# sk4161/EgoScaler

Measured on AMD Instinct MI355X. Metric: clips/sec/GPU (8-frame 224^2, 16-token text) fwd+bwd, higher is better.
Workload: dtype bf16

## Files before the change

egoscaler_amd/csrc/gemm_fast.hip:

```cpp
#include "common.h"
#include <mutex>
#include <queue>
#include <unordered_map>
#include <vector>

#define FT_BK 64

struct FastArgs {
    const bf16_t* A; const bf16_t* B; void* C; const bf16_t* bias; const void* residual;
    int M, N, K;
    long long lda, ldb, ldc, ldr;
    float alpha; int accumulate; int act;
    int tiles_m, tiles_n;
    int splitk; float* ws;
    int full_tm, full_tiles, tail_s;
    int epi; void* C2; long long ldc2;
    int* tickets;
};

typedef __attribute__((address_space(3))) void lds_void;
typedef __attribute__((address_space(1))) const void gbl_void;

__device__ __forceinline__ void glds16(const bf16_t* g, bf16_t* lds_wave_base) {
    __builtin_amdgcn_global_load_lds((gbl_void*)g, (lds_void*)lds_wave_base, 16, 0, 0);
}

template <typename TC, int MT, bool RES, bool ACC>
__device__ __forceinline__ void gemm_epilogue_interior(const FastArgs& g, const f32x4 (&acc)[4][MT], const int mb, const int nb, const int lane) {
    TC* cp = reinterpret_cast<TC*>(g.C) + (long long)(mb + (lane & 15)) * g.ldc + nb + (lane >> 4) * 4;
    const TC* rp = RES ? reinterpret_cast<const TC*>(g.residual) + (long long)(mb + (lane & 15)) * g.ldr + nb + (lane >> 4) * 4 : nullptr;
    const long long cstep = 16 * g.ldc, rstep = 16 * g.ldr;
#pragma unroll
    for (int i = 0; i < MT; ++i) {
#pragma unroll
        for (int j = 0; j < 4; ++j) {
            f32x4 v = acc[j][i];
            if (sizeof(TC) == 2) {
                if (RES) {
                    const u32x2 rr = *reinterpret_cast<const u32x2*>(rp + j * 16);
                    v[0] += __uint_as_float(rr[0] << 16); v[1] += __uint_as_float(rr[0] & 0xFFFF0000u);
// ... 86 lines not shown
                    o[0] = (uint32_t)f2bf(v[0]) | ((uint32_t)f2bf(v[1]) << 16);
                    o[1] = (uint32_t)f2bf(v[2]) | ((uint32_t)f2bf(v[3]) << 16);
                    *reinterpret_cast<u32x2*>(cp) = o;
                } else {
                    f32x4 o = {v[0], v[1], v[2], v[3]};
                    if (rp) o += *reinterpret_cast<const f32x4*>(rp);
                    if (g.accumulate) o += *reinterpret_cast<const f32x4*>(cp);
                    *reinterpret_cast<f32x4*>(cp) = o;
                }
            } else {
#pragma unroll
                for (int r = 0; r < 4; ++r) {
                    if (n + r >= g.N) continue;
                    float x = v[r];
                    if (rp) x += Cvt<TC>::ld(rp + r);
                    if (g.accumulate) x += Cvt<TC>::ld(cp + r);
                    Cvt<TC>::st(cp + r, x);
                }
            }
        }
    }
}

template <typename TC, int BM, int BN, int NS>
__global__ __launch_bounds__((BM / 64) * (BN / 64) * 64, NS == 2 ? 2 : ((BM * BN == 256 * 128) ? 4 : 3))
void gemm_nt_bf16_kernel(FastArgs g) {
    constexpr int MT = 4;
    constexpr int WN = BN / 64, NW = (BM / 64) * WN;
    constexpr int A_PW = BM / 8 / NW, B_PW = BN / 8 / NW;
    constexpr int STAGE = (BM + BN) * FT_BK;
    constexpr bool PF = NS == 2;
    __shared__ __attribute__((aligned(16))) bf16_t smem[NS * STAGE];
    bf16_t* sA = smem;
    bf16_t* sB = smem + BM * FT_BK;
    const int lane = threadIdx.x & 63;
    const int wave = __builtin_amdgcn_readfirstlane(threadIdx.x >> 6);

    const int nwg = g.tiles_m * g.tiles_n;
    int bid = blockIdx.x;
    {
        const int xcd = bid & 7, q = nwg >> 3, r = nwg & 7;
        bid = (xcd < r ? xcd * (q + 1) : r * (q + 1) + (xcd - r) * q) + (bid >> 3);
    }
    const int per_group = 8 * g.tiles_n;
    const int grp = bid / per_group, first_tm = grp * 8;
    const int gsz = (g.tiles_m - first_tm) < 8 ? (g.tiles_m - first_tm) : 8;
// ... 451 lines not shown
                            swiglu_bwd_elem(bf2f(f2bf(v[r])), gv, uv, og[r], ou[r]);
                        }
                        u32x2 o;
                        o[0] = (uint32_t)f2bf(og[0]) | ((uint32_t)f2bf(og[1]) << 16);
                        o[1] = (uint32_t)f2bf(og[2]) | ((uint32_t)f2bf(og[3]) << 16);
                        *reinterpret_cast<u32x2*>(pg) = o;
                        o[0] = (uint32_t)f2bf(ou[0]) | ((uint32_t)f2bf(ou[1]) << 16);
                        o[1] = (uint32_t)f2bf(ou[2]) | ((uint32_t)f2bf(ou[3]) << 16);
                        *reinterpret_cast<u32x2*>(pg + 64) = o;
                    }
#pragma unroll
                for (int it = 0; it < 8; ++it) {
                    const int m = mb + sp * 32 + it * 4 + lr;
                    const u32x4 v = *reinterpret_cast<const u32x4*>(ws3 + (it * 4 + lr) * 272 + ch * 16);
                    if (m < g.M) *reinterpret_cast<u32x4*>(C + (long long)m * g.ldc + 2 * nb + ch * 8) = v;
                }
            }
#undef P8_GU_FETCH
            GSTAMP(4)
            GSTAMP(5)
            GSTAMP_FLUSH
            return;
        }
#pragma unroll
        for (int pass = 0; pass < 2; ++pass) {
#pragma unroll
            for (int ii = 0; ii < 4; ++ii)
#pragma unroll
                for (int j = 0; j < 4; ++j) {
                    const f32x4 v = acc[j][4 * pass + ii];
                    u32x2 o;
                    o[0] = (uint32_t)f2bf(v[0]) | ((uint32_t)f2bf(v[1]) << 16);
                    o[1] = (uint32_t)f2bf(v[2]) | ((uint32_t)f2bf(v[3]) << 16);
                    *reinterpret_cast<u32x2*>(wb + (ii * 16 + (lane & 15)) * 144 + (j * 16 + (lane >> 4) * 4) * 2) = o;
                }
#pragma unroll
            for (int it = 0; it < 8; ++it) {
                const int r = it * 8 + (lane >> 3), ch = lane & 7;
                const u32x4 v = *reinterpret_cast<const u32x4*>(wb + r * 144 + ch * 16);
                const int m = mb + pass * 64 + r;
                if (m < g.M) *reinterpret_cast<u32x4*>(C + (long long)m * g.ldc + nb + ch * 8) = v;
            }
            if (g.epi == 1) {
                bf16_t* C2 = reinterpret_cast<bf16_t*>(g.C2);
#pragma unroll
                for (int ii = 0; ii < 4; ++ii)
#pragma unroll
                    for (int j = 0; j < 2; ++j) {
                        const f32x4 vg = acc[j][4 * pass + ii], vu = acc[j + 2][4 * pass + ii];
                        float o4[4];
#pragma unroll
                        for (int r = 0; r < 4; ++r) {
                            const float gg = bf2f(f2bf(vg[r])), uu = bf2f(f2bf(vu[r]));
                            const float a = bf2f(f2bf(gg * (1.0f / (1.0f + __expf(-gg)))));
                            o4[r] = a * uu;
                        }
                        u32x2 o;
                        o[0] = (uint32_t)f2bf(o4[0]) | ((uint32_t)f2bf(o4[1]) << 16);
// ... 282 lines not shown
                            swiglu_bwd_elem(bf2f(f2bf(v[r])), gv, uv, og[r], ou[r]);
                        }
                        u32x2 o;
                        o[0] = (uint32_t)f2bf(og[0]) | ((uint32_t)f2bf(og[1]) << 16);
                        o[1] = (uint32_t)f2bf(og[2]) | ((uint32_t)f2bf(og[3]) << 16);
                        *reinterpret_cast<u32x2*>(pg) = o;
                        o[0] = (uint32_t)f2bf(ou[0]) | ((uint32_t)f2bf(ou[1]) << 16);
                        o[1] = (uint32_t)f2bf(ou[2]) | ((uint32_t)f2bf(ou[3]) << 16);
                        *reinterpret_cast<u32x2*>(pg + 64) = o;
                    }
                }
#pragma unroll
                for (int it = 0; it < 8; ++it) {
                    if (sp * 32 + it * 4 >= 16 * TL_NB) continue;
                    const int m = mb + sp * 32 + it * 4 + lr;
                    const u32x4 v = *reinterpret_cast<const u32x4*>(ws3 + (it * 4 + lr) * 272 + ch * 16);
                    if (m < g.M) *reinterpret_cast<u32x4*>(C + (long long)m * g.ldc + 2 * nb + ch * 8) = v;
                }
            }
#undef TL_GU_FETCH
            return;
        }
        char* wb = smem + wave * (64 * 144);
#pragma unroll
        for (int pass = 0; pass < 3; ++pass) {
            const int nblk = (TL_NB - 4 * pass) < 4 ? (TL_NB - 4 * pass) : 4;
#pragma unroll
            for (int ii = 0; ii < 4; ++ii) {
                if (ii >= nblk) continue;
#pragma unroll
                for (int j = 0; j < 4; ++j) {
                    const f32x4 v = acc[j][4 * pass + ii];
                    u32x2 o;
                    o[0] = (uint32_t)f2bf(v[0]) | ((uint32_t)f2bf(v[1]) << 16);
                    o[1] = (uint32_t)f2bf(v[2]) | ((uint32_t)f2bf(v[3]) << 16);
                    *reinterpret_cast<u32x2*>(wb + (ii * 16 + (lane & 15)) * 144 + (j * 16 + (lane >> 4) * 4) * 2) = o;
                }
            }
#pragma unroll
            for (int it = 0; it < 8; ++it) {
                const int r = it * 8 + (lane >> 3), ch = lane & 7;
                if (it * 8 >= nblk * 16) continue;
                const u32x4 v = *reinterpret_cast<const u32x4*>(wb + r * 144 + ch * 16);
                const int m = mb + pass * 64 + r;
                const int ncol = TBK ? n0 + 128 * (ch >> 2) + 32 * wc + (ch & 3) * 8 : nb + ch * 8;
                if (m < g.M) *reinterpret_cast<u32x4*>(C + (long long)m * g.ldc + ncol) = v;
            }
            if (g.epi == 1) {
                bf16_t* C2 = reinterpret_cast<bf16_t*>(g.C2);
#pragma unroll
                for (int ii = 0; ii < 4; ++ii) {
                    if (ii >= nblk) continue;
#pragma unroll
                    for (int j = 0; j < 2; ++j) {
                        const f32x4 vg = acc[j][4 * pass + ii], vu = acc[j + 2][4 * pass + ii];
                        float o4[4];
#pragma unroll
                        for (int r = 0; r < 4; ++r) {
                            const float gg = bf2f(f2bf(vg[r])), uu = bf2f(f2bf(vu[r]));
                            const float a = bf2f(f2bf(gg * (1.0f / (1.0f + __expf(-gg)))));
                            o4[r] = a * uu;
// ... 566 lines not shown
    if (sc.P > 0 && sc.Gr > sc.P) sc.Gr = sc.P;
    if (sc.Gr >= 8) sc.Gr &= ~7;
    sc.tickets = (int*)d->workspace;
    sc.slabs = (float*)((char*)d->workspace + 4096);
    return true;
}
static int launch_p8(const egomi_gemm_desc* d, FastArgs& g, const P8Sched& sc, hipStream_t s) {
    g.tiles_m = (d->M + 255) / 256; g.tiles_n = (d->N + 255) / 256;
    g.splitk = 1; g.ws = nullptr; g.full_tm = g.tiles_m; g.full_tiles = g.tiles_m * g.tiles_n; g.tail_s = 1;
    const long long T = (long long)g.tiles_m * g.tiles_n;
    const int grid = T < sc.G ? (sc.Gr > 0 ? sc.Gr : 1) : sc.G;
    if (d->c_dtype == EGOMI_BF16) EGOMI_LAUNCH(gemm_nt_bf16_p8_kernel<bf16_t>, dim3(grid), dim3(512), 0, s, g, sc);
    else if (d->c_dtype == EGOMI_F32) EGOMI_LAUNCH(gemm_nt_bf16_p8_kernel<float>, dim3(grid), dim3(512), 0, s, g, sc);
    else return EGOMI_E_UNSUPPORTED;
    return egomi_launch_status();
}

static int g_tall_mode = -1;
extern "C" int egomi_gemm_set_tall(int mode) { g_tall_mode = mode < 0 ? -1 : (mode > 2 ? 2 : mode); return EGOMI_OK; }
static bool tall_form(const egomi_gemm_desc* d) {
    if (g_tall_mode < 0) { const char* e = getenv("EGOMI_GEMM_TALL"); g_tall_mode = e ? atoi(e) : 1; if (g_tall_mode < 0 || g_tall_mode > 2) g_tall_mode = 1; }
    const int mode = g_tall_mode;
    if (!mode) return false;
    if (d->epilogue != EGOMI_EPI_NONE && d->epilogue != EGOMI_EPI_SLABS && d->epilogue != EGOMI_EPI_SWIGLU && d->epilogue != EGOMI_EPI_SWIGLU_BWD) return false;
    if ((d->M & 7) || (d->N & 7) || d->M < TL_BM || d->N < 256 || d->K < 2048 || d->split_k > 1) return false;
    if ((long long)d->M * d->lda >= (1ll << 31) || (long long)d->N * d->ldb >= (1ll << 31)) return false;
    if (d->c_dtype != EGOMI_BF16 && d->c_dtype != EGOMI_F32) return false;
    if (mode == 2) return true;
    const int ncu = p8_cus();
    const long long tn = (d->N + 255) / 256;
    const long long t256 = (long long)((d->M + 255) / 256) * tn, t352 = (long long)((d->M + TL_BM - 1) / TL_BM) * tn;
    const int rem = (int)(t256 % ncu);
    const double c256 = (double)(t256 / ncu) + (rem ? (rem * 2 <= ncu && d->workspace ? 0.28 + 0.85 * rem / ncu : 1.0) : 0.0);
    const double c352 = 1.31 * (double)((t352 + ncu - 1) / ncu);
    return c352 < 0.98 * c256;
}
static int launch_tall(const egomi_gemm_desc* d, FastArgs& g, hipStream_t s, hipEvent_t t0, hipEvent_t t1) {
    g.tiles_m = (d->M + TL_BM - 1) / TL_BM; g.tiles_n = (d->N + 255) / 256;
    g.splitk = 1; g.ws = nullptr; g.tickets = nullptr;
    if (g.epi == EGOMI_EPI_SLABS) g.epi = 0;
    static int gdepth = -1;
    if (gdepth < 0) { const char* e = getenv("EGOMI_TALL_GROUP"); gdepth = e ? atoi(e) : 8; if (gdepth < 1) gdepth = 8; }
    g.full_tm = gdepth;
    const int nwg = g.tiles_m * g.tiles_n;
    if (t0) (void)hipEventRecord(t0, s);
    if (d->c_dtype == EGOMI_BF16) EGOMI_LAUNCH((gemm_nt_bf16_tall_kernel<bf16_t, false>), dim3(nwg), dim3(512), 0, s, g);
    else EGOMI_LAUNCH((gemm_nt_bf16_tall_kernel<float, false>), dim3(nwg), dim3(512), 0, s, g);
// ... 147 lines not shown
    const int esz = d->c_dtype == EGOMI_BF16 ? 2 : 4;
    egomi_gemm_desc d1 = *d;
    d1.N = Na;
    FastArgs g1 = g;
    g1.N = Na;
    int rc = launch_tall(&d1, g1, s, t0, nullptr);
    if (rc != EGOMI_OK) return rc;
    egomi_gemm_desc d2 = *d;
    FastArgs g2 = g;
    d2.N = g2.N = d->N - Na;
    d2.B = g2.B = (const bf16_t*)d->B + (long long)Na * d->ldb;
    const long long ccol = d->epilogue == EGOMI_EPI_SWIGLU_BWD ? 2ll * Na : (long long)Na;
    d2.C = g2.C = (char*)d->C + ccol * esz;
    if (d->residual) d2.residual = g2.residual = (const char*)d->residual + (long long)Na * esz;
    if (d->epilogue == EGOMI_EPI_SWIGLU) d2.C2 = g2.C2 = (char*)d->C2 + (long long)(Na / 2) * 2;
    if (d->epilogue == EGOMI_EPI_SWIGLU_BWD) d2.C2 = g2.C2 = (char*)d->C2 + 2ll * Na * 2;
    return launch_8phase(&d2, g2, s, nullptr, nullptr, t1);
}

static bool slabs_form_ok(const egomi_gemm_desc* d) {
    return !d->bias && !d->residual && !d->accumulate && d->act == 0 && d->alpha == 1.0f && d->workspace && d->M <= 512 && (d->N & 3) == 0;
}

extern thread_local hipEvent_t egomi_time_start_, egomi_time_stop_;

int egomi_gemm_fast_try(const egomi_gemm_desc* d0, hipStream_t s) {
    const hipEvent_t t0 = egomi_time_start_, t1 = egomi_time_stop_;
    egomi_time_start_ = egomi_time_stop_ = nullptr;
    if (!fast_applicable(d0)) return 1;
    egomi_gemm_desc dl = *d0;
    const egomi_gemm_desc* d = &dl;
    FastArgs g;
    g.A = (const bf16_t*)d->A; g.B = (const bf16_t*)d->B; g.C = d->C; g.bias = (const bf16_t*)d->bias; g.residual = d->residual;
    g.M = d->M; g.N = d->N; g.K = d->K; g.lda = d->lda; g.ldb = d->ldb; g.ldc = d->ldc; g.ldr = d->ldr;
    g.alpha = d->alpha; g.accumulate = d->accumulate; g.act = d->act; g.tickets = nullptr;
    g.epi = d->epilogue; g.C2 = d->C2; g.ldc2 = d->ldc2;
    const int tc = tile_choice(d);
    if (tc == 8 && (d->epilogue == EGOMI_EPI_NONE || d->epilogue == EGOMI_EPI_SLABS) && tall_form(d)) {
        if (d->epilogue == EGOMI_EPI_SLABS && (d->bias || d->accumulate || d->act != 0 || d->alpha != 1.0f || d->c_dtype != EGOMI_BF16)) return EGOMI_E_UNSUPPORTED;
        return launch_tall(d, g, s, t0, t1);
    }
    if (d->epilogue == EGOMI_EPI_SLABS && tc == 8) {
        if (d->bias || d->accumulate || d->act != 0 || d->alpha != 1.0f || d->c_dtype != EGOMI_BF16 || (d->N & 7) ||
            (long long)d->M * d->lda >= (1ll << 31) || (long long)d->N * d->ldb >= (1ll << 31)) return EGOMI_E_UNSUPPORTED;
        if (dl.ws_tickets_zeroed && dl.workspace) {
            if (dl.workspace_bytes > 4096) { dl.workspace = (char*)dl.workspace + 4096; dl.workspace_bytes -= 4096; }
            else { dl.workspace = nullptr; dl.workspace_bytes = 0; }
        }
        g.epi = 0;
        return launch_8phase(d, g, s, nullptr, t0, t1, true);
    }
    if (d->epilogue == EGOMI_EPI_SLABS) {
        if (!slabs_form_ok(d) || tc != 1) return EGOMI_E_UNSUPPORTED;
        if (dl.ws_tickets_zeroed && dl.workspace) {
            if (dl.workspace_bytes > 4096) { dl.workspace = (char*)dl.workspace + 4096; dl.workspace_bytes -= 4096; }
            else return EGOMI_E_UNSUPPORTED;
        }
        g.epi = 0;
        return launch_fast<128, 128>(d, g, s);
    }
// ... 34 lines not shown
```

egoscaler_amd/decode.py:

```python
import ctypes
import os

import torch

from . import lora, ops
from ._lib import c_p, c_i, c_f, c_i64, call
from .ops import P, S, dt


def kv_append(k, v, ld, kc, vc, B, Sq, H, hd, Smax, pos0):
    call("egomi_kv_append", P(k), P(v), c_i64(ld), P(kc), P(vc), c_i(B), c_i(Sq), c_i(H), c_i(hd), c_i(Smax), c_i(pos0), c_i(dt(k.dtype)), S())


def attn_decode(q, ld_q, kc, vc, key_mask, out, B, H, hd, Smax, T_len, scale):
    call("egomi_attn_decode", P(q), c_i64(ld_q), P(kc), P(vc), P(key_mask), c_i64(key_mask.stride(0) if key_mask is not None else 0),
         P(out), c_i64(out.stride(0)), c_i(B), c_i(H), c_i(hd), c_i(Smax), c_i(T_len), c_f(scale), c_i(dt(q.dtype)), S())


def kv_append_fp8(k, v, ld, kc, vc, ks, vs, B, Sq, H, hd, Smax, pos0):
    call("egomi_kv_append_fp8", P(k), P(v), c_i64(ld), P(kc), P(vc), P(ks), P(vs), c_i(B), c_i(Sq), c_i(H), c_i(hd), c_i(Smax), c_i(pos0),
         c_i(dt(k.dtype)), S())


def attn_decode_fp8(q, ld_q, kc, vc, ks, vs, key_mask, out, B, H, hd, Smax, T_len, scale):
    call("egomi_attn_decode_fp8", P(q), c_i64(ld_q), P(kc), P(vc), P(ks), P(vs), P(key_mask), c_i64(key_mask.stride(0) if key_mask is not None else 0),
         P(out), c_i64(out.stride(0)), c_i(B), c_i(H), c_i(hd), c_i(Smax), c_i(T_len), c_f(scale), c_i(dt(q.dtype)), S())


def kv8_quantize(x):
    x = x.float()
# ... 283 lines not shown
        if seed is None:
            seed = int(torch.randint(0, 2 ** 62, (1,)).item())
        self.rng.copy_(torch.tensor([int(seed), 0], dtype=torch.int64))
        self.done_buf.zero_()
        self.done = self.done_buf if eos is not None else None
        kw = dict(repetition_penalty=float(repetition_penalty or 1.0), temperature=float(temperature or 1.0), top_k=int(top_k or 0),
                  top_p=float(1.0 if top_p is None else top_p), do_sample=bool(do_sample), rng=self.rng, eos=eos, pad=pad)

        def steps():
            for t in range(T_new):
                sample_rows(self.lg, sc_buf[t], self.seq, S0 + t, 0, self.tok.view(-1), self.done, draw=t, **kw)
                if t + 1 < T_new:
                    self.step(S0 + t)
        if not use_graph:
            steps()
        else:
            key = (S0, T_new, kw["repetition_penalty"], kw["temperature"], kw["top_k"], kw["top_p"], kw["do_sample"], eos, pad)
            g = self._graphs.get(key)
            if g is None:
                g = torch.cuda.CUDAGraph()
                side = torch.cuda.Stream()
                side.wait_stream(torch.cuda.current_stream())
                with torch.cuda.stream(side):
                    with torch.cuda.graph(g, stream=side):
                        steps()
                torch.cuda.current_stream().wait_stream(side)
                self._graphs[key] = g
            g.replay()
            self.graph = g
        self.pos = S0 + T_new
        return self.seq, sc_buf

    def greedy(self, T_new, use_graph=True, keep_scores=True):
        S0 = self.pos
        scores = [] if keep_scores else None
        if not use_graph:
            for t in range(T_new):
                if keep_scores:
                    scores.append(self.lg.float().clone())
                argmax_rows(self.lg, self.tok.view(-1), self.seq, S0 + t)
                if t + 1 < T_new:
                    self.step(S0 + t)
            self.pos = S0 + T_new
            return self.seq, scores
        sc_buf = torch.zeros(T_new, self.B, self.lg.shape[1], dtype=torch.float32, device=self.eng.device) if keep_scores else None
        g = torch.cuda.CUDAGraph()
        side = torch.cuda.Stream()
        side.wait_stream(torch.cuda.current_stream())
        with torch.cuda.stream(side):
            with torch.cuda.graph(g, stream=side):
                for t in range(T_new):
                    if keep_scores:
                        ops.cast(self.lg, torch.float32, out=sc_buf[t])
                    argmax_rows(self.lg, self.tok.view(-1), self.seq, S0 + t)
                    if t + 1 < T_new:
                        self.step(S0 + t)
        torch.cuda.current_stream().wait_stream(side)
        g.replay()
        self.graph = g
        self.pos = S0 + T_new
        return self.seq, ([sc_buf[t] for t in range(T_new)] if keep_scores else None)

    def _beam_buffers(self):
        R, Smax, dev = self.B, self.Smax, self.eng.device
        z = lambda *s, dtype: torch.zeros(*s, dtype=dtype, device=dev)
        self.kv_row = z(R, Smax, dtype=torch.int32)
        self.fin_seq = z(R, Smax, dtype=torch.int64)
        self.bidx = z(R, Smax, dtype=torch.int32)
        self.fin_bidx = z(R, Smax, dtype=torch.int32)
        self.run_score, self.fin_score = z(R, dtype=torch.float32), z(R, dtype=torch.float32)
        self.fin_flag, self.heur = z(R, dtype=torch.int32), z(R // self.nb, dtype=torch.int32)
        self.ctl = z(8, dtype=torch.int32)
        self._cands = {}
# ... 34 lines not shown
        kw = dict(repetition_penalty=float(repetition_penalty or 1.0), temperature=float(temperature or 1.0), top_k=int(top_k or 0),
                  top_p=float(1.0 if top_p is None else top_p), min_keep=max(2, n_eos + 1), do_sample=bool(do_sample))
        es = early_stopping if early_stopping == "never" else bool(early_stopping)

        def steps():
            for t in range(T_new):
                beam_rows(self.lg, nb if t == 0 else 1, R, nb, sc_buf[t], self.seq_buf, S0 + t, rng=self.rng, draw=t, run_score=self.run_score,
                          cand_key=cands[0], cand_score=cands[1], cand_tok=cands[2], ctl=self.ctl, **kw)
                beam_update(Bi, nb, V, cands[0], cands[1], cands[2], S0, S0 + t, max_len, eos, float(length_penalty), es, self.seq_buf,
                            self.fin_seq, self.bidx, self.fin_bidx, self.kv_row, self.run_score, self.fin_score, self.fin_flag, self.heur,
                            self.tok.view(-1), self.ctl)
                if t + 1 < T_new:
                    self.step(S0 + t)
        if not use_graph:
            steps()
        else:
            key = ("beam", S0, T_new, nb, float(length_penalty), es, eos, pad, tuple(sorted(kw.items())))
            g = self._graphs.get(key)
            if g is None:
                g = torch.cuda.CUDAGraph()
                side = torch.cuda.Stream()
                side.wait_stream(torch.cuda.current_stream())
                with torch.cuda.stream(side):
                    with torch.cuda.graph(g, stream=side):
                        steps()
                torch.cuda.current_stream().wait_stream(side)
                self._graphs[key] = g
            g.replay()
            self.graph = g
        self.pos = S0 + T_new
        n_iter = int(self.ctl[1])
        nrs = int(num_return_sequences)
        rows = (torch.arange(Bi, device=dev)[:, None] * nb + torch.arange(nrs, device=dev)[None, :]).reshape(-1)
        bidx = self.fin_bidx[rows, :T_new]
        lgen = int((bidx >= 0).sum(1).max()) if T_new > 0 else 0
        return (self.fin_seq[rows, :S0 + lgen].clone(), self.fin_score[rows].clone(), sc_buf[:n_iter].clone(), bidx[:, :lgen].long())
```

egoscaler_amd/engine.py:

```python
import os
from typing import Dict

import torch

from . import lora, ops
from .config import EgoDims


class Workspace:

    def __init__(self, device):
        self.device = device
        self.bufs: Dict[str, torch.Tensor] = {}

    def get(self, name, shape, dtype, zero=False):
        t = self.bufs.get(name)
        shape = tuple(int(s) for s in shape)
        if t is None or t.shape != shape or t.dtype != dtype:
            t = torch.empty(shape, dtype=dtype, device=self.device)
            self.bufs[name] = t
            if zero:
                t.zero_()
        elif zero:
            t.zero_()
# ... 7 lines not shown
    def __init__(self, dims: EgoDims, params: Dict[str, torch.Tensor], device, dtype):
        self.dims, self.w, self.device, self.dtype = dims, params, device, dtype
        self.ws = Workspace(device)
        self.w8 = None
        self.prepared = False
        self.prepare_epoch = 0
        self.lm_wT, self.lm_wT_stale, self.lm_wT_ver = None, True, None
        self.param_ref = {}
        self.grad_fresh = set()
        self._xt_last = {}
        self.main_grad: Dict[str, torch.Tensor] = {}
        self.layer_flat: Dict[int, torch.Tensor] = {}
        self.trainable: Dict[str, bool] = {}
        self.ctx = None
        self.grad_sync = None
        self.pb_drop_override = None
        self.reduced_grad = {}
        self.layer_offs = {}
        self._direct, self._direct_done = None, set()
        self.layer_final_hook = None
        self.param_events = {}
        self.use_fused_attention = True
        self.use_fused_swiglu = os.environ.get("EGOMI_NO_FUSED_SWIGLU", "0") != "1"
        self.use_tail_fuse = os.environ.get("EGOMI_NO_TAIL_FUSE", "0") != "1"
        self.use_tn = os.environ.get("EGOMI_GEMM_TN", "1") != "0"
        self.pb_trainer = None
        self.defer_splice_check = False
        self.pending_splice = None
        self.pb_train_mode = False
        self.prepared_bn_stale = False
        self.fold_stale = False
        self.lora = None
        self.lora_version = 0
        self._lora_ws = None

    @staticmethod
    def param_group_of(name):
        if name.startswith("model.layers."):
            return int(name.split(".")[2])
        if name == "model.embed_tokens.weight":
            return "embed"
        if name in ("model.norm.weight", "lm_head.weight"):
            return "post"
        return "pre"

    def wait_params(self, key):
# ... 323 lines not shown
            Wl, bl = w[f"model.point_proj.{2 * nh}.weight"], w[f"model.point_proj.{2 * nh}.bias"]
            feats_proj = ops.mm(cur, Wl, bias=bl, out=ws.get("pp_out", (Bc * Pn, d), T))
            sp, err, cloud_idx = ops.splice_scan(input_ids, tok, Pn, Bc)
            pending_err = self._stash_splice_err(err)
            start_pos = sp
            if save:
                ctx["pp_acts"] = acts
        if save:
            ctx["start_pos"], ctx["cloud_idx"], ctx["n_clouds"] = start_pos, cloud_idx, Bc
            ctx["has_points"] = feats_proj is not None
        x = ws.get("x_emb", (B, S, d), T) if not save else torch.empty(B, S, d, dtype=T, device=self.device)
        self.wait_params("embed")
        ops.embed_splice(input_ids, w["model.embed_tokens.weight"], feats_proj, start_pos, Pn, out=x, cloud_idx=cloud_idx)
        x = x.view(M, d)
        key_mask = None
        if attention_mask is not None:
            key_mask = attention_mask.to(device=self.device, dtype=torch.uint8).contiguous()
        scale = hd ** -0.5
        fused = self.use_fused_attention and T == torch.bfloat16 and hd == 128
        defer = self.use_tail_fuse and T == torch.bfloat16
        pend = pend_res = None
        fuse_swiglu = self.use_fused_swiglu and T == torch.bfloat16 and self.gu_il and (2 * Fd) % 256 == 0 and ops.gemm_kernel_id(M, 2 * Fd, d) == 2
        la = self.lora_groups
        for l in range(L):
            p = f"model.layers.{l}."
            self.wait_params(l)
            lT = {}
            for g, ts in la.items():
                shp = (M, len(ts) * self.lora.r)
                lT[g] = torch.empty(shp, dtype=T, device=self.device) if save else ws.get(f"lora_T_{g}", shp, T)
            if save:
                lc = {"x_in": x, "rstd1": torch.empty(M, dtype=torch.float32, device=self.device),
                      "rstd2": torch.empty(M, dtype=torch.float32, device=self.device),
                      "qkv": torch.empty(M, 3 * d, dtype=T, device=self.device),
                      "gu": torch.empty(M, 2 * Fd, dtype=T, device=self.device)}
                keep_in = self.any_layer_trainable
                h = torch.empty(M, d, dtype=T, device=self.device) if (keep_in or "qkv" in la) else ws.get("h", (M, d), T)
                ao = torch.empty(M, d, dtype=T, device=self.device) if (keep_in or fused or "o" in la) else ws.get("ao", (M, d), T)
                h2 = torch.empty(M, d, dtype=T, device=self.device) if (keep_in or "gu" in la) else ws.get("h2", (M, d), T)
                act = torch.empty(M, Fd, dtype=T, device=self.device) if (keep_in or "down" in la) else ws.get("act", (M, Fd), T)
                x_mid = torch.empty(M, d, dtype=T, device=self.device)
                x_out = torch.empty(M, d, dtype=T, device=self.device)
                qkv, gu, rstd1, rstd2 = lc["qkv"], lc["gu"], lc["rstd1"], lc["rstd2"]
            else:
                h, ao, h2, act = ws.get("h", (M, d), T), ws.get("ao", (M, d), T), ws.get("h2", (M, d), T), ws.get("act", (M, Fd), T)
                x_mid, x_out = ws.get("x_mid", (M, d), T), ws.get(f"x_out{l & 1}", (M, d), T)
                qkv, gu, rstd1, rstd2 = ws.get("qkv", (M, 3 * d), T), ws.get("gu", (M, 2 * Fd), T), None, None
            ops.rmsnorm(x, w[p + "input_layernorm.weight"], lm.rms_norm_eps, rstd=rstd1, out=h, tail=pend, tail_residual=pend_res)
            pend = pend_res = None
            t_qkv = None
            if l in self.wqkv:
                if defer and "qkv" not in la:
                    _, t_qkv = ops.mm(h, self.wqkv[l], out=qkv, defer_tail=True)
                else:
                    ops.mm(h, self.wqkv[l], out=qkv)
            else:
                ops.mm(h, w[p + "self_attn.q_proj.weight"], out=qkv[:, :d])
                ops.mm(h, w[p + "self_attn.k_proj.weight"], out=qkv[:, d:2 * d])
                ops.mm(h, w[p + "self_attn.v_proj.weight"], out=qkv[:, 2 * d:])
            if "qkv" in la:
                self._lora_fwd(l, "qkv", h, qkv, lT["qkv"])
            if t_qkv is not None:
                ops.rope_qkv_tail_(qkv, self.cos, self.sin, M, S, past, H, hd, 3 * d, t_qkv)
            else:
                ops.rope_(qkv, self.cos, self.sin, M, S, past, 2 * H, hd, 3 * d)
            if kv_sink is not None:
                kv_sink(l, qkv, B, S)
            lse = None
            if fused:
                Pm = None
                lse = torch.empty(B, H, S, dtype=torch.float32, device=self.device) if save else ws.get("att_lse", (B, H, S), torch.float32)
                ops.attn_fwd(qkv, B, S, H, hd, scale, ao, lse, causal=True, key_mask=key_mask)
            else:
                Pm = self._attention(qkv, B, S, H, hd, ao, True, key_mask, scale, save)
            if defer and "o" not in la:
                _, t_o = ops.mm(ao, w[p + "self_attn.o_proj.weight"], out=x_mid, residual=x, defer_tail=True)
                ops.rmsnorm(x_mid, w[p + "post_attention_layernorm.weight"], lm.rms_norm_eps, rstd=rstd2, out=h2, tail=t_o, tail_residual=x)
            else:
                ops.mm(ao, w[p + "self_attn.o_proj.weight"], out=x_mid, residual=x)
                if "o" in la:
                    self._lora_fwd(l, "o", ao, x_mid, lT["o"])
                ops.rmsnorm(x_mid, w[p + "post_attention_layernorm.weight"], lm.rms_norm_eps, rstd=rstd2, out=h2)
            gu_il = l in self.wgu and self.gu_il
            if gu_il:
                if fuse_swiglu and "gu" not in la:
                    ops.mm(h2, self.wgu[l], out=gu, swiglu_out=act)
                else:
# ... 380 lines not shown
```

egoscaler_amd/ops.py:

```python
import ctypes
import math

import torch

from . import _lib
from ._lib import c_p, c_i, c_d, c_f, c_sz, c_i64, call

F32, BF16 = 0, 1


def dt(t: torch.dtype) -> int:
    if t == torch.float32:
        return F32
    if t == torch.bfloat16:
        return BF16
    raise TypeError(f"unsupported dtype {t}")


def P(t):
    if t is None:
        return c_p(None)
    if not t.is_cuda:
        raise _lib.EgomiError("egoscaler_amd ops need CUDA/HIP tensors (no CPU fallback)")
    return c_p(t.data_ptr())
# ... 75 lines not shown
    call("egomi_fps", P(pts), c_i(B), c_i(N), c_i(C), P(start), c_i(num_group), P(idx), P(cen), S())
    return idx, cen


def knn_group(pts, center, k, out_dtype=torch.float32):
    pts, center = _c(pts, torch.float32), _c(center, torch.float32)
    B, N, C = pts.shape
    G = center.shape[1]
    idx = torch.empty(B, G, k, dtype=torch.int32, device=pts.device)
    nb = torch.empty(B, G, k, C, dtype=out_dtype, device=pts.device)
    call("egomi_knn_group", P(pts), P(center), c_i(B), c_i(N), c_i(C), c_i(G), c_i(k), P(idx), P(nb), c_i(dt(out_dtype)), S())
    return idx, nb


class GemmDesc(ctypes.Structure):
    _fields_ = [("A", c_p), ("B", c_p), ("C", c_p), ("bias", c_p), ("residual", c_p),
                ("M", c_i), ("N", c_i), ("K", c_i),
                ("lda", c_i64), ("ldb", c_i64), ("ldc", c_i64), ("ldr", c_i64),
                ("a_layout", c_i), ("b_layout", c_i), ("ab_dtype", c_i), ("c_dtype", c_i),
                ("batch", c_i), ("batch_inner", c_i),
                ("sA0", c_i64), ("sA1", c_i64), ("sB0", c_i64), ("sB1", c_i64), ("sC0", c_i64), ("sC1", c_i64),
                ("alpha", c_f), ("accumulate", c_i), ("act", c_i), ("force_generic", c_i),
                ("workspace", c_p), ("workspace_bytes", c_i64), ("split_k", c_i), ("ws_tickets_zeroed", c_i),
                ("epilogue", c_i), ("C2", c_p), ("ldc2", c_i64)]


ACT_NONE, ACT_GELU, ACT_RELU = 0, 1, 2


class GemmProfiler:

    def __init__(self, min_flops=1e9, tuned_only=True, kernel_ids=None):
        self.min_flops, self.recs, self.enabled, self.tuned_only = min_flops, [], True, tuned_only
        self.kernel_ids = kernel_ids if kernel_ids is not None else ((1, 2) if tuned_only else None)

    def summary(self):
        torch.cuda.synchronize()
        n, flops, ms, call_ms = 0, 0.0, 0.0, 0.0
        L = _lib.lib()
        for e0, e1, f, k0, k1 in self.recs:
            n += 1
            flops += f
            c = e0.elapsed_time(e1)
            call_ms += c
            if k0 is not None:
                t = ctypes.c_float()
                ms += t.value if L.egomi_event_elapsed_ms(k0, k1, ctypes.byref(t)) == 0 else c
# ... 7 lines not shown
            for _, _, _, k0, k1 in self.recs:
                if k0 is not None:
                    L.egomi_event_destroy(k0)
                    L.egomi_event_destroy(k1)
        except Exception:
            pass


PROFILER = None


_TAIL_WS = {}


def _tail_workspace(device, nbytes=(4096 + 256 * 2 * 262144)):
    ws = _TAIL_WS.get(device)
    if ws is None:
        ws = _TAIL_WS[device] = torch.zeros(nbytes // 4, dtype=torch.float32, device=device)
    return ws


def gemm_raw(A, B, C, M, N, K, lda, ldb, ldc, a_layout=0, b_layout=0, bias=None, residual=None, ldr=0,
             act=0, alpha=1.0, accumulate=False, batch=1, batch_inner=1, strides=(0, 0, 0, 0, 0, 0), force_generic=False,
             workspace=None, split_k=0, persistent=None, swiglu_out=None, slabs=False, count_only=False, defer_tail=False, swiglu_bwd_gu=None):
    if A.dtype != B.dtype:
        raise TypeError("gemm: A and B dtypes differ")
    d = GemmDesc()
    d.A, d.B, d.C = A.data_ptr(), B.data_ptr(), C.data_ptr()
    d.bias = bias.data_ptr() if bias is not None else None
    d.residual = residual.data_ptr() if residual is not None else None
    if bias is not None and bias.dtype != A.dtype:
        raise TypeError("gemm: bias dtype must equal the operand dtype")
    if residual is not None and residual.dtype != C.dtype:
        raise TypeError("gemm: residual dtype must equal the output dtype")
    d.M, d.N, d.K = M, N, K
    d.lda, d.ldb, d.ldc, d.ldr = lda, ldb, ldc, ldr
    d.a_layout, d.b_layout = a_layout, b_layout
    d.ab_dtype, d.c_dtype = dt(A.dtype), dt(C.dtype)
    d.batch, d.batch_inner = batch, batch_inner
    d.sA0, d.sA1, d.sB0, d.sB1, d.sC0, d.sC1 = strides
    d.alpha, d.accumulate, d.act, d.force_generic = alpha, int(accumulate), act, int(force_generic)
    if swiglu_out is not None:
        d.epilogue, d.C2, d.ldc2 = 1, swiglu_out.data_ptr(), _ld(swiglu_out)
    if swiglu_bwd_gu is not None:
        if swiglu_out is not None or swiglu_bwd_gu.dtype != C.dtype:
            raise TypeError("gemm: swiglu_bwd_gu excludes swiglu_out and must have the output dtype")
        d.epilogue, d.C2, d.ldc2 = 3, swiglu_bwd_gu.data_ptr(), _ld(swiglu_bwd_gu)
    if workspace is None and M >= 1024 and batch <= 1:
        workspace = _tail_workspace(A.device)
        if persistent is False:
            workspace = workspace[1024:]
        else:
            d.ws_tickets_zeroed = 2 if persistent else 1
    if workspace is not None:
        d.workspace, d.workspace_bytes, d.split_k = workspace.data_ptr(), workspace.numel() * workspace.element_size(), split_k
    for t in (A, B, C):
        if not t.is_cuda:
            raise _lib.EgomiError("gemm needs device tensors")
    if slabs or count_only:
        d.epilogue = 2
        n = _lib.lib().egomi_gemm_slab_count(ctypes.byref(d))
        if count_only:
            return n
        if n < 2:
            raise _lib.EgomiError("gemm: the library would not split this product (egomi_gemm_slab_count == 0)")
        call("egomi_gemm", ctypes.byref(d), S())
        return n
    tail = None
    if defer_tail and d.workspace and bias is None and act == 0 and alpha == 1.0 and not accumulate and swiglu_out is None and \
            C.dtype == torch.bfloat16:
        row0, slices = c_i(0), c_i(0)
        if _lib.lib().egomi_gemm_tail_plan(ctypes.byref(d), ctypes.byref(row0), ctypes.byref(slices)) == 0 and slices.value >= 2:
            d.epilogue = 2
            if _lib.lib().egomi_gemm_kernel_id(ctypes.byref(d)) == 2:
                tail = (row0.value, slices.value, d.workspace + (4096 if d.ws_tickets_zeroed else 0))
            else:
                d.epilogue = 0
    prof = PROFILER
    flops = 2.0 * M * N * K * max(1, batch)
    kid = _lib.lib().egomi_gemm_kernel_id(ctypes.byref(d)) if (prof is not None and prof.enabled and flops >= prof.min_flops) else None
    if kid is not None and (prof.kernel_ids is None or kid in prof.kernel_ids):
# ... 395 lines not shown
```

include/egomi.h:

```cpp
#ifndef EGOMI_H
#define EGOMI_H
#include <stddef.h>
#include <stdint.h>

#ifdef __cplusplus
extern "C" {
#endif

#define EGOMI_OK 0
#define EGOMI_E_BADARG (-1)
#define EGOMI_E_SHAPE (-2)
#define EGOMI_E_LAUNCH (-3)
#define EGOMI_E_UNSUPPORTED (-4)

#define EGOMI_F32 0
#define EGOMI_BF16 1

typedef void* egomi_stream_t;

int egomi_version(void);
const char* egomi_strerror(int code);
const char* egomi_last_launch_error(void);

size_t egomi_unproject_workspace_bytes(int B, int T, int H, int W);
// ... 9 lines not shown
int egomi_pc_norm(const double* points, const float* colors, float* out, int B, int N, egomi_stream_t stream);

int egomi_fps(const float* pts, int B, int N, int C, const int32_t* start, int G,
              int32_t* out_idx, float* out_center, egomi_stream_t stream);

int egomi_knn_group(const float* pts, const float* center, int B, int N, int C, int G, int K,
                    int32_t* out_idx, void* out_nb, int out_dtype, egomi_stream_t stream);

typedef struct egomi_gemm_desc {
    const void* A; const void* B; void* C; const void* bias; const void* residual;
    int M, N, K;
    int64_t lda, ldb, ldc, ldr;
    int a_layout, b_layout;
    int ab_dtype, c_dtype;
    int batch, batch_inner;
    int64_t sA0, sA1, sB0, sB1, sC0, sC1;
    float alpha;
    int accumulate;
    int act;
    int force_generic;
    void* workspace; int64_t workspace_bytes; int split_k;
    int ws_tickets_zeroed;
    int epilogue; void* C2; int64_t ldc2;
} egomi_gemm_desc;
#define EGOMI_EPI_NONE 0
#define EGOMI_EPI_SWIGLU 1
#define EGOMI_EPI_SLABS 2
#define EGOMI_EPI_SWIGLU_BWD 3
int egomi_gemm(const egomi_gemm_desc* desc, egomi_stream_t stream);
int egomi_gemm_kernel_id(const egomi_gemm_desc* desc);
int egomi_gemm_set_tall(int mode);
int egomi_gemm_slab_count(const egomi_gemm_desc* desc);
int egomi_gemm_tail_plan(const egomi_gemm_desc* desc, int* row0, int* slices);
int egomi_gemm_tn_tail_plan(const egomi_gemm_desc* desc, int* row0, int* slices);
int egomi_event_create(void** event);
int egomi_event_destroy(void* event);
int egomi_event_elapsed_ms(void* start, void* stop, float* ms);
int egomi_gemm_time_next(void* start, void* stop);

typedef struct egomi_attn_desc {
    const void* q; const void* k; const void* v; void* o; float* lse;
    const void* dout; float* delta; void* dq; void* dk; void* dv;
    const uint8_t* key_mask;
    int B, H, S, head_dim;
    int64_t ld_qkv, ld_o, ld_dqkv;
    float scale;
    int causal;
    int dtype;
    const float* rope_cos; const float* rope_sin;
} egomi_attn_desc;
int egomi_attn_fwd(const egomi_attn_desc* desc, egomi_stream_t stream);
// ... 149 lines not shown
```

Before: 63.85.

## Fuse rotary embedding into the QKV GEMM epilogue

Adds a RoPE epilogue to the 8-phase and tall bf16 GEMM kernels. Each block stages its output strips in LDS, loads the cos/sin rows, and writes the rotated Q/K columns directly, so the separate rope_ kernel pass over qkv is skipped when the fused path qualifies. The engine turns this on by default for bf16 with head_dim 128 and no qkv LoRA. A query call checks eligibility before launch. The change also disables Python GC while CUDA graphs are captured in decode. Costs are extra barriers and register pressure in the epilogue, plus the loss of the deferred-tail path for qkv when rope fusion is chosen.

Result: no change. 63.85 (median of 6 runs) (-0.0%).

```diff
diff --git a/egoscaler_amd/csrc/gemm_fast.hip b/egoscaler_amd/csrc/gemm_fast.hip
--- a/egoscaler_amd/csrc/gemm_fast.hip
+++ b/egoscaler_amd/csrc/gemm_fast.hip
@@ -16,6 +16,8 @@
     int full_tm, full_tiles, tail_s;
     int epi; void* C2; long long ldc2;
     int* tickets;
+    const float* rope_cos; const float* rope_sin;
+    int rope_cols, rope_seq, rope_pos;
 };
 
 typedef __attribute__((address_space(3))) void lds_void;
@@ -148,6 +150,68 @@
     }
 }
 
+#define ROPE_STRIP_BYTES (64 * 144)
+struct RopeTab { u32x4 c[2], s[2]; };
+__device__ __forceinline__ uint32_t bf_pair(float lo, float hi) { return (uint32_t)f2bf(lo) | ((uint32_t)f2bf(hi) << 16); }
+__device__ __forceinline__ void rope_tab_load(const FastArgs& g, int mrow, int nrows, int wc, int lane, RopeTab& t) {
+    if (wc * 16 >= nrows) return;
+    f32x4 c[2][2], s[2][2];
+#pragma unroll
+    for (int it = 0; it < 2; ++it) {
+        int m = mrow + wc * 16 + it * 8 + (lane >> 3);
+        m = m < g.M ? m : g.M - 1;
+        const long long off = (long long)(g.rope_pos + m % g.rope_seq) * 64 + (lane & 7) * 8;
+        c[it][0] = *reinterpret_cast<const f32x4*>(g.rope_cos + off); c[it][1] = *reinterpret_cast<const f32x4*>(g.rope_cos + off + 4);
+        s[it][0] = *reinterpret_cast<const f32x4*>(g.rope_sin + off); s[it][1] = *reinterpret_cast<const f32x4*>(g.rope_sin + off + 4);
+    }
+#pragma unroll
+    for (int it = 0; it < 2; ++it)
+#pragma unroll
+        for (int q = 0; q < 4; ++q) {
+            t.c[it][q] = bf_pair(c[it][q >> 1][2 * (q & 1)], c[it][q >> 1][2 * (q & 1) + 1]);
+            t.s[it][q] = bf_pair(s[it][q >> 1][2 * (q & 1)], s[it][q >> 1][2 * (q & 1) + 1]);
+        }
+}
+__device__ __forceinline__ float bf_lo(uint32_t v) { return __uint_as_float(v << 16); }
+__device__ __forceinline__ float bf_hi(uint32_t v) { return __uint_as_float(v & 0xFFFF0000u); }
+__device__ __forceinline__ void rope_strip_store(const FastArgs& g, const char* strips, int mrow, int nrows, int n0, int wc, int lane, const RopeTab& t) {
+    if (wc * 16 >= nrows) return;
+    bf16_t* C = reinterpret_cast<bf16_t*>(g.C);
+    const int ch = lane & 7;
+#pragma unroll
+    for (int it = 0; it < 2; ++it) {
+        const int r = wc * 16 + it * 8 + (lane >> 3), m = mrow + r;
+#pragma unroll
+        for (int h = 0; h < 2; ++h) {
+            const u32x4 av = *reinterpret_cast<const u32x4*>(strips + (2 * h) * ROPE_STRIP_BYTES + r * 144 + ch * 16);
+            const u32x4 bv = *reinterpret_cast<const u32x4*>(strips + (2 * h + 1) * ROPE_STRIP_BYTES + r * 144 + ch * 16);
+            u32x4 oa, ob;
+#pragma unroll
+            for (int q = 0; q < 4; ++q) {
+                float xa[2], xb[2];
+#pragma unroll
+                for (int e = 0; e < 2; ++e) {
+                    const float a = e ? bf_hi(av[q]) : bf_lo(av[q]), b = e ? bf_hi(bv[q]) : bf_lo(bv[q]);
+                    const float c = e ? bf_hi(t.c[it][q]) : bf_lo(t.c[it][q]), s = e ? bf_hi(t.s[it][q]) : bf_lo(t.s[it][q]);
+                    xa[e] = bf2f(f2bf(a * c)) + bf2f(f2bf(-b * s));
+                    xb[e] = bf2f(f2bf(b * c)) + bf2f(f2bf(a * s));
+                }
+                oa[q] = bf_pair(xa[0], xa[1]); ob[q] = bf_pair(xb[0], xb[1]);
+            }
+            if (m < g.M) {
+                bf16_t* p = C + (long long)m * g.ldc + n0 + 128 * h + ch * 8;
+                *reinterpret_cast<u32x4*>(p) = oa;
+                *reinterpret_cast<u32x4*>(p + 64) = ob;
+            }
+        }
+    }
+}
+#define ROPE_PASS(mrow_, nrows_) { \
+        RopeTab rt_; rope_tab_load(g, (mrow_), (nrows_), wc, lane, rt_); \
+        asm volatile("s_waitcnt lgkmcnt(0)" ::: "memory"); __builtin_amdgcn_s_barrier(); \
+        rope_strip_store(g, smem_c + wr * 4 * ROPE_STRIP_BYTES, (mrow_), (nrows_), n0, wc, lane, rt_); \
+        asm volatile("s_waitcnt lgkmcnt(0)" ::: "memory"); __builtin_amdgcn_s_barrier(); }
+
 template <typename TC, int BM, int BN, int NS>
 __global__ __launch_bounds__((BM / 64) * (BN / 64) * 64, NS == 2 ? 2 : ((BM * BN == 256 * 128) ? 4 : 3))
 void gemm_nt_bf16_kernel(FastArgs g) {
@@ -645,6 +709,8 @@
             GSTAMP_FLUSH
             return;
         }
+        const bool rope = g.epi == 4 && n0 < g.rope_cols;
+        const char* smem_c = reinterpret_cast<const char*>(smem);
 #pragma unroll
         for (int pass = 0; pass < 2; ++pass) {
 #pragma unroll
@@ -657,6 +723,7 @@
                     o[1] = (uint32_t)f2bf(v[2]) | ((uint32_t)f2bf(v[3]) << 16);
                     *reinterpret_cast<u32x2*>(wb + (ii * 16 + (lane & 15)) * 144 + (j * 16 + (lane >> 4) * 4) * 2) = o;
                 }
+            if (rope) { ROPE_PASS(mb + pass * 64, 64) continue; }
 #pragma unroll
             for (int it = 0; it < 8; ++it) {
                 const int r = it * 8 + (lane >> 3), ch = lane & 7;
@@ -985,6 +1052,8 @@
             return;
         }
         char* wb = smem + wave * (64 * 144);
+        const bool rope = !TBK && g.epi == 4 && n0 < g.rope_cols;
+        const char* smem_c = smem;
 #pragma unroll
         for (int pass = 0; pass < 3; ++pass) {
             const int nblk = (TL_NB - 4 * pass) < 4 ? (TL_NB - 4 * pass) : 4;
@@ -1000,6 +1069,7 @@
                     *reinterpret_cast<u32x2*>(wb + (ii * 16 + (lane & 15)) * 144 + (j * 16 + (lane >> 4) * 4) * 2) = o;
                 }
             }
+            if (rope) { ROPE_PASS(mb + pass * 64, nblk * 16) continue; }
 #pragma unroll
             for (int it = 0; it < 8; ++it) {
                 const int r = it * 8 + (lane >> 3), ch = lane & 7;
@@ -1612,7 +1682,8 @@
     if (g_tall_mode < 0) { const char* e = getenv("EGOMI_GEMM_TALL"); g_tall_mode = e ? atoi(e) : 1; if (g_tall_mode < 0 || g_tall_mode > 2) g_tall_mode = 1; }
     const int mode = g_tall_mode;
     if (!mode) return false;
-    if (d->epilogue != EGOMI_EPI_NONE && d->epilogue != EGOMI_EPI_SLABS && d->epilogue != EGOMI_EPI_SWIGLU && d->epilogue != EGOMI_EPI_SWIGLU_BWD) return false;
+    if (d->epilogue != EGOMI_EPI_NONE && d->epilogue != EGOMI_EPI_SLABS && d->epilogue != EGOMI_EPI_SWIGLU && d->epilogue != EGOMI_EPI_SWIGLU_BWD &&
+        d->epilogue != EGOMI_EPI_ROPE) return false;
     if ((d->M & 7) || (d->N & 7) || d->M < TL_BM || d->N < 256 || d->K < 2048 || d->split_k > 1) return false;
     if ((long long)d->M * d->lda >= (1ll << 31) || (long long)d->N * d->ldb >= (1ll << 31)) return false;
     if (d->c_dtype != EGOMI_BF16 && d->c_dtype != EGOMI_F32) return false;
@@ -1806,6 +1877,30 @@
     return !d->bias && !d->residual && !d->accumulate && d->act == 0 && d->alpha == 1.0f && d->workspace && d->M <= 512 && (d->N & 3) == 0;
 }
 
+static int rope_form(const egomi_gemm_desc* d0) {
+    if (!fast_applicable(d0)) return 0;
+    egomi_gemm_desc dl = *d0;
+    dl.epilogue = EGOMI_EPI_ROPE;
+    const egomi_gemm_desc* d = &dl;
+    if (d->force_generic || tile_choice(d) != 8 || d->c_dtype != EGOMI_BF16) return 0;
+    if (d->bias || d->residual || d->accumulate || d->act != 0 || d->alpha != 1.0f) return 0;
+    if ((d->N & 255) || d->rope_cols <= 0 || (d->rope_cols & 255) || d->rope_cols > d->N || (d->ldc & 7) || ((uintptr_t)d->C & 15)) return 0;
+    if (!d->rope_cos || !d->rope_sin || (((uintptr_t)d->rope_cos | (uintptr_t)d->rope_sin) & 15) || d->rope_seq <= 0 || d->rope_pos < 0 ||
+        (long long)d->rope_pos + (d->M < d->rope_seq ? d->M : d->rope_seq) > d->rope_tab_rows) return 0;
+    if ((long long)d->M * d->lda >= (1ll << 31) || (long long)d->N * d->ldb >= (1ll << 31)) return 0;
+    if (dl.ws_tickets_zeroed && dl.workspace) {
+        if (dl.workspace_bytes > 4096) { dl.workspace = (char*)dl.workspace + 4096; dl.workspace_bytes -= 4096; }
+        else { dl.workspace = nullptr; dl.workspace_bytes = 0; }
+    }
+    if (tall_form(d)) return 1;
+    egomi_gemm_desc dp = *d0, dps = dl;
+    dp.epilogue = dps.epilogue = EGOMI_EPI_NONE;
+    P8Sched sc;
+    if (split_cols(&dps) || p8_applicable(&dp, sc)) return 0;
+    return tail_plan_for(d).rows == 0 ? 2 : 0;
+}
+extern "C" int egomi_gemm_rope_ok(const egomi_gemm_desc* d) { return d && rope_form(d) ? 1 : 0; }
+
 extern thread_local hipEvent_t egomi_time_start_, egomi_time_stop_;
 
 int egomi_gemm_fast_try(const egomi_gemm_desc* d0, hipStream_t s) {
@@ -1820,6 +1915,17 @@
     g.alpha = d->alpha; g.accumulate = d->accumulate; g.act = d->act; g.tickets = nullptr;
     g.epi = d->epilogue; g.C2 = d->C2; g.ldc2 = d->ldc2;
     const int tc = tile_choice(d);
+    if (d->epilogue == EGOMI_EPI_ROPE) {
+        const int form = rope_form(d0);
+        if (!form) return EGOMI_E_UNSUPPORTED;
+        g.rope_cos = d->rope_cos; g.rope_sin = d->rope_sin; g.rope_cols = d->rope_cols; g.rope_seq = d->rope_seq; g.rope_pos = d->rope_pos;
+        if (form == 1) return launch_tall(d, g, s, t0, t1);
+        if (dl.ws_tickets_zeroed && dl.workspace) {
+            if (dl.workspace_bytes > 4096) { dl.workspace = (char*)dl.workspace + 4096; dl.workspace_bytes -= 4096; }
+            else { dl.workspace = nullptr; dl.workspace_bytes = 0; }
+        }
+        return launch_8phase(d, g, s, nullptr, t0, t1);
+    }
     if (tc == 8 && (d->epilogue == EGOMI_EPI_NONE || d->epilogue == EGOMI_EPI_SLABS) && tall_form(d)) {
         if (d->epilogue == EGOMI_EPI_SLABS && (d->bias || d->accumulate || d->act != 0 || d->alpha != 1.0f || d->c_dtype != EGOMI_BF16)) return EGOMI_E_UNSUPPORTED;
         return launch_tall(d, g, s, t0, t1);
diff --git a/egoscaler_amd/decode.py b/egoscaler_amd/decode.py
--- a/egoscaler_amd/decode.py
+++ b/egoscaler_amd/decode.py
@@ -1,4 +1,6 @@
+import contextlib
 import ctypes
+import gc
 import os
 
 import torch
@@ -6,6 +8,19 @@
 from . import lora, ops
 from ._lib import c_p, c_i, c_f, c_i64, call
 from .ops import P, S, dt
+
+
+@contextlib.contextmanager
+def _capture(g, stream):
+    gc.collect()
+    enabled = gc.isenabled()
+    gc.disable()
+    try:
+        with torch.cuda.graph(g, stream=stream):
+            yield
+    finally:
+        if enabled:
+            gc.enable()
 
 
 def kv_append(k, v, ld, kc, vc, B, Sq, H, hd, Smax, pos0):
@@ -335,7 +350,7 @@
                 side = torch.cuda.Stream()
                 side.wait_stream(torch.cuda.current_stream())
                 with torch.cuda.stream(side):
-                    with torch.cuda.graph(g, stream=side):
+                    with _capture(g, side):
                         steps()
                 torch.cuda.current_stream().wait_stream(side)
                 self._graphs[key] = g
@@ -361,7 +376,7 @@
         side = torch.cuda.Stream()
         side.wait_stream(torch.cuda.current_stream())
         with torch.cuda.stream(side):
-            with torch.cuda.graph(g, stream=side):
+            with _capture(g, side):
                 for t in range(T_new):
                     if keep_scores:
                         ops.cast(self.lg, torch.float32, out=sc_buf[t])
@@ -442,7 +457,7 @@
                 side = torch.cuda.Stream()
                 side.wait_stream(torch.cuda.current_stream())
                 with torch.cuda.stream(side):
-                    with torch.cuda.graph(g, stream=side):
+                    with _capture(g, side):
                         steps()
                 torch.cuda.current_stream().wait_stream(side)
                 self._graphs[key] = g
diff --git a/egoscaler_amd/engine.py b/egoscaler_amd/engine.py
--- a/egoscaler_amd/engine.py
+++ b/egoscaler_amd/engine.py
@@ -53,6 +53,7 @@
         self.param_events = {}
         self.use_fused_attention = True
         self.use_fused_swiglu = os.environ.get("EGOMI_NO_FUSED_SWIGLU", "0") != "1"
+        self.use_rope_fuse = os.environ.get("EGOMI_ROPE_FUSE", "1") != "0"
         self.use_tail_fuse = os.environ.get("EGOMI_NO_TAIL_FUSE", "0") != "1"
         self.use_tn = os.environ.get("EGOMI_GEMM_TN", "1") != "0"
         self.pb_trainer = None
@@ -422,6 +423,8 @@
         pend = pend_res = None
         fuse_swiglu = self.use_fused_swiglu and T == torch.bfloat16 and self.gu_il and (2 * Fd) % 256 == 0 and ops.gemm_kernel_id(M, 2 * Fd, d) == 2
         la = self.lora_groups
+        fuse_rope = save and self.use_rope_fuse and T == torch.bfloat16 and hd == 128 and "qkv" not in la
+        rope_epi = (self.cos, self.sin, S, past, 2 * d)
         for l in range(L):
             p = f"model.layers.{l}."
             self.wait_params(l)
@@ -448,9 +451,12 @@
                 qkv, gu, rstd1, rstd2 = ws.get("qkv", (M, 3 * d), T), ws.get("gu", (M, 2 * Fd), T), None, None
             ops.rmsnorm(x, w[p + "input_layernorm.weight"], lm.rms_norm_eps, rstd=rstd1, out=h, tail=pend, tail_residual=pend_res)
             pend = pend_res = None
-            t_qkv = None
+            t_qkv, roped = None, False
             if l in self.wqkv:
-                if defer and "qkv" not in la:
+                if fuse_rope and ops.mm(h, self.wqkv[l], out=qkv, rope=rope_epi, rope_query=True):
+                    ops.mm(h, self.wqkv[l], out=qkv, rope=rope_epi)
+                    roped = True
+                elif defer and "qkv" not in la:
                     _, t_qkv = ops.mm(h, self.wqkv[l], out=qkv, defer_tail=True)
                 else:
                     ops.mm(h, self.wqkv[l], out=qkv)
@@ -462,7 +468,7 @@
                 self._lora_fwd(l, "qkv", h, qkv, lT["qkv"])
             if t_qkv is not None:
                 ops.rope_qkv_tail_(qkv, self.cos, self.sin, M, S, past, H, hd, 3 * d, t_qkv)
-            else:
+            elif not roped:
                 ops.rope_(qkv, self.cos, self.sin, M, S, past, 2 * H, hd, 3 * d)
             if kv_sink is not None:
                 kv_sink(l, qkv, B, S)
diff --git a/egoscaler_amd/ops.py b/egoscaler_amd/ops.py
--- a/egoscaler_amd/ops.py
+++ b/egoscaler_amd/ops.py
@@ -121,7 +121,8 @@
                 ("sA0", c_i64), ("sA1", c_i64), ("sB0", c_i64), ("sB1", c_i64), ("sC0", c_i64), ("sC1", c_i64),
                 ("alpha", c_f), ("accumulate", c_i), ("act", c_i), ("force_generic", c_i),
                 ("workspace", c_p), ("workspace_bytes", c_i64), ("split_k", c_i), ("ws_tickets_zeroed", c_i),
-                ("epilogue", c_i), ("C2", c_p), ("ldc2", c_i64)]
+                ("epilogue", c_i), ("C2", c_p), ("ldc2", c_i64),
+                ("rope_cos", c_p), ("rope_sin", c_p), ("rope_cols", c_i), ("rope_seq", c_i), ("rope_pos", c_i), ("rope_tab_rows", c_i)]
 
 
 ACT_NONE, ACT_GELU, ACT_RELU = 0, 1, 2
@@ -175,7 +176,8 @@
 
 def gemm_raw(A, B, C, M, N, K, lda, ldb, ldc, a_layout=0, b_layout=0, bias=None, residual=None, ldr=0,
              act=0, alpha=1.0, accumulate=False, batch=1, batch_inner=1, strides=(0, 0, 0, 0, 0, 0), force_generic=False,
-             workspace=None, split_k=0, persistent=None, swiglu_out=None, slabs=False, count_only=False, defer_tail=False, swiglu_bwd_gu=None):
+             workspace=None, split_k=0, persistent=None, swiglu_out=None, slabs=False, count_only=False, defer_tail=False, swiglu_bwd_gu=None,
+             rope=None, rope_query=False):
     if A.dtype != B.dtype:
         raise TypeError("gemm: A and B dtypes differ")
     d = GemmDesc()
@@ -199,6 +201,14 @@
         if swiglu_out is not None or swiglu_bwd_gu.dtype != C.dtype:
             raise TypeError("gemm: swiglu_bwd_gu excludes swiglu_out and must have the output dtype")
         d.epilogue, d.C2, d.ldc2 = 3, swiglu_bwd_gu.data_ptr(), _ld(swiglu_bwd_gu)
+    if rope is not None:
+        if swiglu_out is not None or swiglu_bwd_gu is not None or defer_tail or slabs or count_only:
+            raise TypeError("gemm: rope excludes the other epilogues")
+        cos, sin, seq, pos, cols = rope
+        if cos.dtype != torch.float32 or sin.shape != cos.shape or cos.dim() != 2 or cos.shape[1] != 64 or not (cos.is_contiguous() and sin.is_contiguous()):
+            raise TypeError("gemm: rope tables must be contiguous fp32 [rows, 64]")
+        d.epilogue, d.rope_cos, d.rope_sin = 4, cos.data_ptr(), sin.data_ptr()
+        d.rope_cols, d.rope_seq, d.rope_pos, d.rope_tab_rows = cols, seq, pos, cos.shape[0]
     if workspace is None and M >= 1024 and batch <= 1:
         workspace = _tail_workspace(A.device)
         if persistent is False:
@@ -210,6 +220,8 @@
     for t in (A, B, C):
         if not t.is_cuda:
             raise _lib.EgomiError("gemm needs device tensors")
+    if rope_query:
+        return bool(_lib.lib().egomi_gemm_rope_ok(ctypes.byref(d)))
     if slabs or count_only:
         d.epilogue = 2
         n = _lib.lib().egomi_gemm_slab_count(ctypes.byref(d))
diff --git a/include/egomi.h b/include/egomi.h
--- a/include/egomi.h
+++ b/include/egomi.h
@@ -55,11 +55,15 @@
     void* workspace; int64_t workspace_bytes; int split_k;
     int ws_tickets_zeroed;
     int epilogue; void* C2; int64_t ldc2;
+    const float* rope_cos; const float* rope_sin;
+    int rope_cols, rope_seq, rope_pos, rope_tab_rows;
 } egomi_gemm_desc;
 #define EGOMI_EPI_NONE 0
 #define EGOMI_EPI_SWIGLU 1
 #define EGOMI_EPI_SLABS 2
 #define EGOMI_EPI_SWIGLU_BWD 3
+#define EGOMI_EPI_ROPE 4
+int egomi_gemm_rope_ok(const egomi_gemm_desc* desc);
 int egomi_gemm(const egomi_gemm_desc* desc, egomi_stream_t stream);
 int egomi_gemm_kernel_id(const egomi_gemm_desc* desc);
 int egomi_gemm_set_tall(int mode);
```
